# divideon/xvc

Hardware: AMD Instinct MI355X
Metric: hot-path frame passes/s (TZ + sub-pel ME, MC, transform + RDOQ + dequant + inverse, deblock, pad, PSNR parts), bit-exact vs the reference's classes (higher is better)
Workload: dtype u16; 1 GPU; 1920x1080 yuv420p 30fps synthetic, QP 32, internal bitdepth 10, 16x16 CUs, TZ range 96, RDOQ (RdoQuant::QuantRdo + CoeffSignHideRdo, picture-initial CABAC contexts); cus_per_picture=8160, parallelism=3 independent picture chains in flight

## Files before the change

### include/xvcgpu.h

```cpp
#ifndef XVCGPU_H_
#define XVCGPU_H_

#include "xvcgpu_types.h"

#ifdef __cplusplus
extern "C" {
#endif

typedef enum xvcgpu_status {
  XVCGPU_OK = 0,
  XVCGPU_INVALID_ARGUMENT = 10,
  XVCGPU_NO_DEVICE = 20,
  XVCGPU_OUT_OF_MEMORY = 30,
  XVCGPU_DEVICE_ERROR = 40,
  XVCGPU_UNSUPPORTED = 50
} xvcgpu_status;

typedef struct xvcgpu_ctx xvcgpu_ctx;
typedef struct xvcgpu_picture xvcgpu_picture;

xvcgpu_status xvcgpu_create(int device, xvcgpu_ctx **out);
void xvcgpu_destroy(xvcgpu_ctx *ctx);
const char *xvcgpu_last_error(const xvcgpu_ctx *ctx);
const char *xvcgpu_version(void);
// ... 146 lines not shown
                                  const xvcgpu_mc_lic_block *d_blocks, int n);

xvcgpu_status xvcgpu_inter_pred_batch(xvcgpu_ctx *ctx, const xvcgpu_picture *const *refs,
                                      int n_refs, const xvcgpu_picture *rec,
                                      xvcgpu_picture *pred,
                                      const xvcgpu_inter_block *d_blocks, int n);

xvcgpu_status xvcgpu_inter_pred_batch_to(xvcgpu_ctx *ctx, const xvcgpu_picture *const *refs,
                                         int n_refs, const xvcgpu_picture *rec,
                                         xvcgpu_picture *scratch,
                                         const xvcgpu_inter_block *d_blocks,
                                         const xvcgpu_block_pos *d_dst, int n);

xvcgpu_status xvcgpu_copy_blocks(xvcgpu_ctx *ctx, const xvcgpu_picture *src,
                                 xvcgpu_picture *dst, const xvcgpu_copy_block *d_blocks,
                                 int n);

xvcgpu_status xvcgpu_inv_transform_cu_order(xvcgpu_ctx *ctx, xvcgpu_picture *rec,
                                            const xvcgpu_tx_block *d_blocks, int n_cus,
                                            const int16_t *d_levels,
                                            const uint32_t *d_level_offsets,
                                            const int32_t *d_nnz);

xvcgpu_status xvcgpu_mc_affine_batch(xvcgpu_ctx *ctx, const xvcgpu_picture *ref,
                                     xvcgpu_picture *pred,
                                     const xvcgpu_mc_affine_block *d_blocks, int n);

xvcgpu_status xvcgpu_mc_bipred_batch(xvcgpu_ctx *ctx, const xvcgpu_picture *ref0,
                                     const xvcgpu_picture *ref1,
                                     xvcgpu_picture *pred,
                                     const xvcgpu_mc_bi_block *d_blocks, int n);

xvcgpu_status xvcgpu_bipred_search(xvcgpu_ctx *ctx, const xvcgpu_picture *orig,
                                   const xvcgpu_picture *ref_other,
                                   const xvcgpu_picture *ref_search,
                                   const xvcgpu_bi_block *d_jobs, int n,
                                   xvcgpu_me_result *d_results,
                                   int max_block_size);
xvcgpu_status xvcgpu_bipred_search_lic(xvcgpu_ctx *ctx, const xvcgpu_picture *orig,
                                       const xvcgpu_picture *ref_other,
                                       const xvcgpu_picture *ref_search,
                                       const xvcgpu_picture *rec,
                                       const xvcgpu_bi_block *d_jobs,
                                       const xvcgpu_mc_lic_block *d_neighbours, int n,
                                       xvcgpu_me_result *d_results, int max_block_size);

// ... 54 lines not shown
                                          xvcgpu_cu_info *d_cus);
xvcgpu_status xvcgpu_fwd_from_me_classify_prove(
    xvcgpu_ctx *ctx, const xvcgpu_picture *orig, const xvcgpu_picture *ref, xvcgpu_picture *pred,
    const xvcgpu_me_block *d_blocks, const xvcgpu_me_result *d_results, int n, int qp_y, int qp_c,
    int ref_poc, int16_t *d_coeffs, const uint32_t *d_coeff_offsets, size_t n_coeffs,
    int16_t *d_levels, int32_t *d_nnz, xvcgpu_cu_info *d_cus,
    const xvcgpu_rdoq_contexts *d_contexts, const xvcgpu_rdoq_params *d_params);
xvcgpu_status xvcgpu_quant_rdo_classified_batch(xvcgpu_ctx *ctx, int bitdepth,
                                                const xvcgpu_tx_block *d_blocks, int n,
                                                const int16_t *d_coeffs,
                                                const uint32_t *d_offsets, size_t n_coeffs,
                                                int16_t *d_levels, int32_t *d_nnz,
                                                const xvcgpu_rdoq_contexts *d_contexts,
                                                const xvcgpu_rdoq_params *d_params,
                                                xvcgpu_cu_info *d_cus);

xvcgpu_status xvcgpu_quant_rdo_reserve(xvcgpu_ctx *ctx, int n, size_t n_coeffs);

#define XVCGPU_PROVE_ZERO_AUTO_BLOCKS 65536
#define XVCGPU_PROVE_ZERO_AUTO_QP 30
xvcgpu_status xvcgpu_quant_rdo_set_prove_zero(xvcgpu_ctx *ctx, int mode);

xvcgpu_status xvcgpu_quant_rdo_class_counts(xvcgpu_ctx *ctx, int32_t out[3]);
xvcgpu_status xvcgpu_quant_rdo_set_four_lane_only(xvcgpu_ctx *ctx, int on);

xvcgpu_status xvcgpu_recon_from_me(xvcgpu_ctx *ctx, const xvcgpu_picture *orig,
                                   const xvcgpu_picture *ref, xvcgpu_picture *rec,
                                   const xvcgpu_me_block *d_blocks,
                                   const xvcgpu_me_result *d_results, int n,
                                   int qp_y, int qp_c, int intra_pic, int ref_poc,
                                   int32_t *d_nnz, xvcgpu_cu_info *d_cus);

xvcgpu_status xvcgpu_fwd_from_me(xvcgpu_ctx *ctx, const xvcgpu_picture *orig,
                                 const xvcgpu_picture *ref, xvcgpu_picture *pred,
                                 const xvcgpu_me_block *d_blocks,
                                 const xvcgpu_me_result *d_results, int n, int16_t *d_coeffs,
                                 const uint32_t *d_coeff_offsets);
xvcgpu_status xvcgpu_recon_from_me_rdoq(xvcgpu_ctx *ctx, const xvcgpu_picture *orig,
                                        const xvcgpu_picture *ref, xvcgpu_picture *rec,
                                        const xvcgpu_me_block *d_blocks,
                                        const xvcgpu_me_result *d_results, int n,
                                        int qp_y, int qp_c, int tx_flags, int ref_poc,
                                        int32_t *d_nnz, xvcgpu_cu_info *d_cus,
                                        const xvcgpu_rdoq_contexts *d_contexts,
                                        const xvcgpu_rdoq_params *d_params);

// ... 202 lines not shown
```

### xvc_amd/api.py

```python
import ctypes as C
import os

import numpy as np

HERE = os.path.dirname(os.path.abspath(__file__))
LIB_PATH = os.environ.get("XVCGPU_LIB") or os.path.join(HERE, "libxvcgpu.so")

BORDER_LUMA = 128
BORDER_CHROMA = 64
ME_FULLPEL = 1
ME_SUBPEL = 2
ME_LIC_JOBS = 4
ME_HINT_SQ16 = 8
ME_ONLY_SQ16 = 16

METRIC_SSD, METRIC_SATD, METRIC_SATD_ACONLY, METRIC_SAD, METRIC_SAD_FAST, \
    METRIC_SAD_ACONLY, METRIC_SAD_ACONLY_FAST, METRIC_STRUCTURAL_SSD = range(8)
TX_DEFAULT, TX_DCT2, TX_DCT5, TX_DCT8, TX_DST1, TX_DST7 = range(6)

CU_DTYPE = np.dtype([("x", "<u2"), ("y", "<u2"), ("w", "u1"), ("h", "u1"),
                     ("intra", "u1"), ("cbf_luma", "u1"), ("qp_y", "i1"),
                     ("qp_c", "i1"), ("ref_idx0", "i1"), ("reserved", "i1"),
                     ("ref_poc", "<i4", (2,)), ("mv", "<i4", (2, 4, 2))])
ME_DTYPE = np.dtype([("x", "<i2"), ("y", "<i2"), ("w", "u1"), ("h", "u1"),
# ... 129 lines not shown
    "xvcgpu_picture_download", "xvcgpu_picture_upload_padded",
    "xvcgpu_picture_download_padded", "xvcgpu_picture_plane",
    "xvcgpu_picture_copy", "xvcgpu_pad_border", "xvcgpu_metric_batch", "xvcgpu_mc_metric_batch",
    "xvcgpu_me_search", "xvcgpu_me_search_sized", "xvcgpu_mc_batch", "xvcgpu_mc_from_me",
    "xvcgpu_mc_bipred_batch", "xvcgpu_bipred_search", "xvcgpu_mc_affine_batch", "xvcgpu_mc_lic_batch",
    "xvcgpu_affine_me_batch",
    "xvcgpu_me_search_refs",
    "xvcgpu_bipred_search_refs",
    "xvcgpu_mc_metric_batch_refs",
    "xvcgpu_affine_me_batch_refs",
    "xvcgpu_cu_info_from_me", "xvcgpu_recon_from_me", "xvcgpu_residual_batch",
    "xvcgpu_fwd_transform_batch", "xvcgpu_inv_transform_batch",
    "xvcgpu_deblock", "xvcgpu_deblock_rows", "xvcgpu_deblock_pad_ssd", "xvcgpu_picture_ssd", "xvcgpu_picture_ssd_rows",
    "xvcgpu_picture_import", "xvcgpu_picture_export", "xvcgpu_picture_crc",
    "xvcgpu_variance_map", "xvcgpu_histogram_distance",
    "xvcgpu_intra_pred_batch", "xvcgpu_intra_satd_batch", "xvcgpu_intra_recon_batch",
    "xvcgpu_intra_select_modes", "xvcgpu_frame_pass", "xvcgpu_frame_pass_multi", "xvcgpu_copy_segments",
    "xvcgpu_get_transform_matrix", "xvcgpu_inter_pred_batch", "xvcgpu_deblock_tree",
    "xvcgpu_residual_rdoq_batch", "xvcgpu_quant_rdo_batch", "xvcgpu_recon_from_me_rdoq",
    "xvcgpu_quant_rdo_reserve", "xvcgpu_quant_rdo_class_counts", "xvcgpu_quant_rdo_set_prove_zero",
    "xvcgpu_tx_eval_batch", "xvcgpu_root_cbf_batch", "xvcgpu_bipred_search_lic",
    "xvcgpu_inter_pred_batch_to", "xvcgpu_copy_blocks", "xvcgpu_intra_recon_waves",
    "xvcgpu_host_alloc", "xvcgpu_host_free", "xvcgpu_memcpy_h2d_async",
    "xvcgpu_inv_transform_cu_order",
    "xvcgpu_fwd_from_me_classify", "xvcgpu_fwd_from_me_classify_prove", "xvcgpu_quant_rdo_classified_batch",
    "xvcgpu_event_create", "xvcgpu_event_destroy", "xvcgpu_event_record", "xvcgpu_event_wait",
    "xvcgpu_event_synchronize", "xvcgpu_comm_unique_id", "xvcgpu_comm_create",
    "xvcgpu_comm_destroy", "xvcgpu_comm_world", "xvcgpu_comm_rank", "xvcgpu_comm_wait_event",
    "xvcgpu_comm_record_event", "xvcgpu_comm_sync", "xvcgpu_comm_group_begin",
    "xvcgpu_comm_group_end", "xvcgpu_comm_send_picture", "xvcgpu_comm_recv_picture",
    "xvcgpu_comm_send_rows", "xvcgpu_comm_recv_rows", "xvcgpu_comm_all_reduce_sum_u64",
    "xvcgpu_comm_send_bytes", "xvcgpu_comm_recv_bytes", "xvcgpu_inv_transform_dist_batch",
    "xvcgpu_fwd_from_me", "xvcgpu_output_bytes", "xvcgpu_picture_convert_to",
    "xvcgpu_me_plan_create", "xvcgpu_me_plan_counts", "xvcgpu_me_plan_destroy",
    "xvcgpu_me_search_planned", "xvcgpu_frame_pass_planned",
]

_vp = C.c_void_p
_pd = C.c_ssize_t
_lib = None


class XvcGpuError(RuntimeError):
    pass


class MePlan:
# ... 105 lines not shown
        "xvcgpu_intra_pred_batch": [_vp, _vp, _vp, _vp, C.c_int],
        "xvcgpu_intra_satd_batch": [_vp, _vp, _vp, _vp, C.c_int, _vp, C.c_int],
        "xvcgpu_intra_recon_batch": [_vp, _vp, _vp, _vp, _vp, C.c_int, _vp, _vp, _vp],
        "xvcgpu_intra_select_modes": [_vp, _vp, _vp, C.c_int, _vp, _vp, _vp, C.c_int],
        "xvcgpu_frame_pass": [_vp, C.POINTER(FramePassArgs), C.c_int],
        "xvcgpu_frame_pass_multi": [C.POINTER(_vp), C.POINTER(C.POINTER(FramePassArgs)), C.c_int,
                                    C.c_int],
        "xvcgpu_copy_segments": [_vp, _vp, C.c_int],
        "xvcgpu_get_transform_matrix": [C.c_int, C.c_int, _vp],
        "xvcgpu_inter_pred_batch": [_vp, C.POINTER(_vp), C.c_int, _vp, _vp, _vp, C.c_int],
        "xvcgpu_residual_rdoq_batch": [_vp, _vp, _vp, _vp, _vp, C.c_int, _vp, _vp, _vp, _vp, _vp],
        "xvcgpu_recon_from_me_rdoq": [_vp, _vp, _vp, _vp, _vp, _vp, C.c_int, C.c_int, C.c_int,
                                      C.c_int, C.c_int, _vp, _vp, _vp, _vp],
        "xvcgpu_quant_rdo_reserve": [_vp, C.c_int, C.c_size_t],
        "xvcgpu_quant_rdo_class_counts": [_vp, _vp],
        "xvcgpu_quant_rdo_set_prove_zero": [_vp, C.c_int],
        "xvcgpu_quant_rdo_set_four_lane_only": [_vp, C.c_int],
        "xvcgpu_tx_eval_batch": [_vp, _vp, C.c_int, _vp, _vp],
        "xvcgpu_inter_pred_batch_to": [_vp, _vp, C.c_int, _vp, _vp, _vp, _vp, C.c_int],
        "xvcgpu_copy_blocks": [_vp, _vp, _vp, _vp, C.c_int],
        "xvcgpu_host_alloc": [_vp, C.c_size_t, C.POINTER(_vp)],
        "xvcgpu_host_free": [_vp, _vp],
        "xvcgpu_inv_transform_cu_order": [_vp, _vp, _vp, C.c_int, _vp, _vp, _vp],
        "xvcgpu_memcpy_h2d_async": [_vp, _vp, _vp, C.c_size_t],
        "xvcgpu_memcpy_d2h_async": [_vp, _vp, _vp, C.c_size_t],
        "xvcgpu_upload_ahead": [_vp, _vp, _vp, C.c_size_t, _vp, _vp],
        "xvcgpu_eval_dist_batch": [_vp, _vp, _vp, _vp, C.c_int, _vp, C.c_int, _vp],
        "xvcgpu_cs_start_fold": [_vp, _vp, C.c_int, C.c_int, _vp, _vp, _vp, _vp, _vp, C.c_int, C.c_int],
        "xvcgpu_cs_uni_fold": [_vp, _vp, C.c_int, C.c_int, _vp, _vp, _vp, _vp, _vp],
        "xvcgpu_cs_bi_fold": [_vp, _vp, C.c_int, C.c_int, _vp, _vp, _vp, _vp],
        "xvcgpu_cs_merge_fold": [_vp, _vp, C.c_int, C.c_int, _vp, _vp, _vp, _vp],
        "xvcgpu_residual_rdoq_batch_at": [_vp, _vp, _vp, _vp, _vp, C.c_int, _vp, _vp, _vp, _vp, _vp, _vp,
                                          C.c_int, _vp, C.c_int, _vp],
        "xvcgpu_intra_recon_waves": [_vp, _vp, _vp, _vp, _vp, _vp, C.c_int, _vp, _vp, _vp],
        "xvcgpu_bipred_search_lic": [_vp, _vp, _vp, _vp, _vp, _vp, _vp, C.c_int, _vp, C.c_int],
        "xvcgpu_root_cbf_batch": [_vp, _vp, C.c_int, _vp],
        "xvcgpu_quant_rdo_batch": [_vp, C.c_int, _vp, C.c_int, _vp, _vp, C.c_size_t, _vp, _vp,
                                   _vp, _vp],
        "xvcgpu_deblock_pad_ssd": [_vp, _vp, _vp, _vp, _vp, C.c_int, _vp, C.c_int, C.c_int,
                                   C.c_int, C.c_int, C.c_int, _vp],
        "xvcgpu_deblock_tree": [_vp, _vp, _vp, C.c_int, _vp, C.c_int, C.c_int, C.c_int,
                                C.c_int, C.c_int, C.c_int],
        "xvcgpu_event_create": [_vp, C.POINTER(_vp)],
        "xvcgpu_event_record": [_vp, _vp],
        "xvcgpu_event_wait": [_vp, _vp],
        "xvcgpu_event_synchronize": [_vp],
# ... 882 lines not shown
```

### xvc_amd/csrc/k_multi.h

```cpp
#ifndef XVCGPU_K_MULTI_H_
#define XVCGPU_K_MULTI_H_

#include "k_me2.h"
#include "k_misc.h"
#include "k_rdoq.h"
#include "k_recon.h"
#include "k_tail.h"
#include "k_tx.h"
#include "k_tx2.h"

struct ReconMultiArgs {
  PicView orig, ref, rec;
  const xvcgpu_me_block *blocks;
  const xvcgpu_me_result *results;
  int n_cus, qp_y, qp_c, ref_poc;
  int32_t *nnz_out;
  xvcgpu_cu_info *cus;
  int16_t *coeffs;
  const uint32_t *coeff_off;
};
template <bool FWD>
__global__ void __launch_bounds__(256)
recon_from_me_multi_kernel(MultiArgs<ReconMultiArgs> m, const int16_t *tx_tables,
                           const int16_t *tx_tables_t, TxTableLayout lay) {
// ... 4 lines not shown
                                        FwdClassify());
}

struct RdoqMultiArgs {
  const xvcgpu_tx_block *blocks;
  int n;
  const int16_t *coeffs;
  const uint32_t *d_off;
  int16_t *levels;
  int32_t *nnz_out;
  RdoqLists l;
  const xvcgpu_rdoq_contexts *rq_ctx;
  const xvcgpu_rdoq_params *rq_prm;
};
__global__ void __launch_bounds__(256)
rdoq_classify_multi_kernel(MultiArgs<RdoqMultiArgs> m, int bd) {
  const RdoqMultiArgs &a = m.a[blockIdx.y];
  rdoq_classify_kernel_body(bd, a.blocks, a.n, a.coeffs, a.d_off, a.levels, a.nnz_out, a.l);
}
__global__ void __launch_bounds__(1024)
rdoq_compact_multi_kernel(MultiArgs<RdoqMultiArgs> m) {
  const RdoqMultiArgs &a = m.a[blockIdx.y];
  rdoq_compact_kernel_body(a.n, a.l);
}
__global__ void __launch_bounds__(64, RDOQ4_MIN_WAVES)
quant_rdo_packed4_multi_kernel(MultiArgs<RdoqMultiArgs> m, int bd, int g16) {
  const RdoqMultiArgs &a = m.a[blockIdx.y];
  quant_rdo_packed4_kernel_body(bd, a.blocks, a.l, g16, a.coeffs, a.d_off, a.levels, a.nnz_out,
                                a.rq_ctx, a.rq_prm, nullptr);
}
__global__ void __launch_bounds__(64, RDOQ_MIN_WAVES)
quant_rdo_packed_multi_kernel(MultiArgs<RdoqMultiArgs> m, int bd) {
  const RdoqMultiArgs &a = m.a[blockIdx.y];
  quant_rdo_packed_kernel_body(bd, a.blocks, a.l, a.coeffs, a.d_off, a.levels, a.nnz_out,
                               a.rq_ctx, a.rq_prm, nullptr);
}

struct InvMultiArgs {
  PicView pred, rec;
  const xvcgpu_tx_block *blocks;
  int n;
  int16_t *levels;
  const uint32_t *level_off;
  int32_t *nnz;
};
__global__ void __launch_bounds__(64 * TX2_WAVES)
// ... 49 lines not shown
```

### xvc_amd/csrc/k_rdoq.h

```cpp
#ifndef XVCGPU_K_RDOQ_H_
#define XVCGPU_K_RDOQ_H_

#include "dev_common.h"
#include "dev_tables.h"
#include "k_me.h"
#include "k_me2.h"
#include "xvcgpu_internal.h"

__constant__ uint32_t kEntropyBits[128] = {
#include "entropy_bits.inc"
};

#define RQ_BYPASS 32768u
__device__ uint32_t gEntropyBits[128];

#ifdef XVCGPU_TRACE
__device__ unsigned long long g_rq_trace[4096][16];
#define RQ_TRACE(k)                                                          \
  do {                                                                       \
    if (threadIdx.x == 0 && blockIdx.x < 4096)                               \
      g_rq_trace[blockIdx.x][k] = __builtin_amdgcn_s_memtime();              \
  } while (0)
#define RQ_TRACE_RT(k)                                                       \
  do {                                                                       \
// ... 1362 lines not shown
    }
  }
}

__global__ void __launch_bounds__(1024)
rdoq_count_kernel(int n, RdoqLists l) {
  __shared__ int wsum[3][16];
  int cnt[3];
  rdoq_chunk_counts(n, l, cnt);
  const int t = threadIdx.x;
#pragma unroll
  for (int k = 0; k < 3; k++) {
    const int v = wave_reduce_add_i32(cnt[k]);
    if ((t & 63) == 0) wsum[k][t >> 6] = v;
  }
  __syncthreads();
  if (t < 3) {
    int v = 0;
    for (int w = 0; w < 16; w++) v += wsum[t][w];
    l.part[4 * blockIdx.x + t] = v;
  }
}

__global__ void __launch_bounds__(1024)
rdoq_scatter_kernel(int n, RdoqLists l) {
  __shared__ int part[3][1024];
  __shared__ int base[3];
  const int t = threadIdx.x, b = blockIdx.x;
  {
    int v[3] = {0, 0, 0};
    for (int j = t; j < b; j += 1024) {
      v[0] += l.part[4 * j];
      v[1] += l.part[4 * j + 1];
      v[2] += l.part[4 * j + 2];
    }
#pragma unroll
    for (int k = 0; k < 3; k++) {
      const int w = wave_reduce_add_i32(v[k]);
      if ((t & 63) == 0) part[k][t >> 6] = w;
    }
    __syncthreads();
    if (t < 3) {
      int sum = 0;
      for (int w = 0; w < 16; w++) sum += part[t][w];
      base[t] = sum;
    }
    __syncthreads();
  }
  int cnt[3];
  rdoq_chunk_counts(n, l, cnt);
  int inc[3];
#pragma unroll
  for (int k = 0; k < 3; k++) {
    int v = cnt[k];
#pragma unroll
    for (int d = 1; d < 64; d <<= 1) {
      const int o = __shfl_up(v, d, 64);
// ... 15 lines not shown
#pragma unroll
      for (int d = 1; d < 16; d <<= 1) {
        const int o = __shfl_up(v, d, 64);
        if (t >= d) v += o;
      }
      if (t < 16) part[k][16 + t] = v;
    }
  }
  __syncthreads();
  const int bs[3] = {b0, b1, b2};
  int pos[3];
#pragma unroll
  for (int k = 0; k < 3; k++)
    pos[k] = bs[k] + inc[k] - cnt[k] + ((t >> 6) ? part[k][16 + (t >> 6) - 1] : 0);
  const int i = b * RDOQ_CHUNK + 4 * t;
  if (i < n) {
    const uint32_t v = reinterpret_cast<const uint32_t *>(l.cls)[i >> 2];
#pragma unroll
    for (int k = 0; k < 4; k++) {
      const int c = (int)(signed char)(v >> (8 * k));
      if (i + k < n && c >= 0) l.list[c][pos[c]++] = i + k;
    }
  }
  if (b == (int)gridDim.x - 1 && t == 1023)
    for (int k = 0; k < 3; k++) l.count[k] = bs[k] + part[k][16 + 15];
}

template <int G, int NSB>
struct RdoqPackedLds {
  static constexpr int GROUPS = 64 / G;
  static constexpr int MAXC = 16 * NSB;
  static constexpr int MAXSB = NSB;
  static constexpr int MAXR = RQ_PADDED(MAXC);
  static constexpr int MAXT = RQ_CF_PADDED(MAXC);
  alignas(8) long long sb_code_cost[GROUPS][MAXSB];
  alignas(8) int16_t cf[GROUPS][MAXT], lv[GROUPS][MAXT];
  alignas(8) int16_t wl[GROUPS][RQ_WL(MAXC)];
  long long fcs[NSB == 64 ? 256 : 1];
  unsigned short rate_up[GROUPS][MAXR];
  alignas(8) unsigned ctx_bits[2 * sizeof(xvcgpu_rdoq_contexts)];
  unsigned csbf_bits[GROUPS][MAXSB];
  unsigned char csbf[GROUPS][MAXSB], sb_live[GROUPS][MAXSB], sb_dcz[GROUPS][MAXSB];
  unsigned char sb_of_scan[GROUPS][NSB == 4 ? MAXSB : MAXSB * 4];
  unsigned lp_bits[32];
};

struct RqTileCf {
  const int16_t *p;
// ... 273 lines not shown
```

### xvc_amd/csrc/k_tx2.h

```cpp
#ifndef XVCGPU_K_TX2_H_
#define XVCGPU_K_TX2_H_

#include "dev_common.h"
#include "dev_tables.h"
#include "k_me.h"
#include "k_me2.h"
#include "k_tx.h"
#include "xvcgpu_internal.h"

#define TX2_WAVES 4

typedef short tx2_v2s __attribute__((ext_vector_type(2)));

struct __attribute__((aligned(16))) Tx2Shared {
  int16_t r[256];
  int16_t t[256];
  int16_t c[256];
};

__device__ __forceinline__ int tx2_dot2(uint32_t a, uint32_t b, int acc) {
  return __builtin_amdgcn_sdot2(__builtin_bit_cast(tx2_v2s, a),
                                __builtin_bit_cast(tx2_v2s, b), acc, false);
}

// ... 395 lines not shown
  if (job >= n) return;
  const int ci = job >> 1;
  if (!(job & 1)) {
    const int bi = 3 * ci;
    if (nnz_out[bi] == 0) return;
    const xvcgpu_tx_block b = blocks[bi];
    if (!tx_small_job(b)) return;
    const PlaneView pc = rec.c[0];
    tx2_job<TX_MODE_INV, 64, false>(s, b, bi, rec.bd, pc, pc.p + (ptrdiff_t)b.y * pc.stride + b.x,
                                    pc.stride, pc, levels, level_off, nnz_out, tx_tables,
                                    tx_tables_t, lay);
    return;
  }
  if (nnz_out[3 * ci + 1] == 0 && nnz_out[3 * ci + 2] == 0) return;
  const int g = ME2_LANE >> 5, bi = 3 * ci + 1 + g;
  const xvcgpu_tx_block b = blocks[bi];
  if (!tx_small_job(b) || b.w * b.h > 64) return;
  const PlaneView pc = g ? rec.c[2] : rec.c[1];
  tx2_job<TX_MODE_INV, 32, false>(s, b, bi, rec.bd, pc, pc.p + (ptrdiff_t)b.y * pc.stride + b.x,
                                  pc.stride, pc, levels, level_off, nnz_out, tx_tables,
                                  tx_tables_t, lay, nullptr, g * 128);
}

template <int MODE, bool RDOQ = false>
__global__ void __launch_bounds__(64 * TX2_WAVES)
residual_wave_kernel(PicView orig, PicView pred, PicView rec, const xvcgpu_tx_block *blocks, int n, int16_t *levels, const uint32_t *level_off, int32_t *nnz_out, const int16_t *tx_tables, const int16_t *tx_tables_t, TxTableLayout lay, const xvcgpu_rdoq_contexts *rq_ctx = nullptr, const xvcgpu_rdoq_params *rq_prm = nullptr, unsigned long long *dist_out = nullptr) {
  residual_wave_kernel_body<MODE, RDOQ>(orig, pred, rec, blocks, n, levels, level_off, nnz_out, tx_tables, tx_tables_t, lay, rq_ctx, rq_prm, dist_out);
}

template <int MODE, bool RDOQ>
__device__ __forceinline__ void
residual_cu_body(const PicView &orig, const PicView &pred, const PicView &rec, const xvcgpu_tx_block *blocks, int n,
                   int16_t *levels, const uint32_t *level_off, int32_t *nnz_out,
                   const int16_t *tx_tables, const int16_t *tx_tables_t, TxTableLayout lay,
                   const xvcgpu_rdoq_contexts *rq_ctx, const xvcgpu_rdoq_params *rq_prm,
                   const xvcgpu_block_pos *src_pos, const xvcgpu_eval_cand *ecands, int n_head,
                   uint64_t *eout, int strength) {
  struct Big {
    TxShared s;
    RdoqShared<RDOQ ? 1024 : 4> rq;
  };
  struct Small {
    Tx2Shared s;
    RdoqShared<256> rq;
  };
  constexpr size_t kBytes = sizeof(Big) > sizeof(Small) ? sizeof(Big) : sizeof(Small);
// ... 65 lines not shown
```

### xvc_amd/csrc/xvcgpu.hip

```cpp
#include <hip/hip_runtime.h>
#include <stdlib.h>
#include <stdio.h>
#include <string.h>

#include <algorithm>
#include <new>
#include <vector>

#include "k_deblock.h"
#include "k_tail.h"
#include "k_me.h"
#include "k_me2.h"
#include "k_me_plan.h"
#include "k_metric.h"
#include "k_misc.h"
#include "k_pad.h"
#include "k_tx.h"
#include "k_tx2.h"
#include "k_recon.h"
#include "k_bipred.h"
#include "k_stats.h"
#include "k_output.h"
#include "k_intra.h"
#include "k_affine_me.h"
// ... 1349 lines not shown
}

xvcgpu_status xvcgpu_quant_rdo_set_four_lane_only(xvcgpu_ctx *ctx, int on) {
  if (!ctx) return XVCGPU_INVALID_ARGUMENT;
  ctx->rdoq_four_lane_only = on ? 1 : 0;
  return XVCGPU_OK;
}

xvcgpu_status xvcgpu_quant_rdo_reserve(xvcgpu_ctx *ctx, int n, size_t n_coeffs) {
  if (!ctx || n < 0) return XVCGPU_INVALID_ARGUMENT;
  return ensure_rdoq_scratch(ctx, n, n_coeffs);
}

static RdoqLists rdoq_lists_of(xvcgpu_ctx *ctx) {
  const int cap = ctx->rdoq_lists_cap;
  RdoqLists l;
  l.count = ctx->d_rdoq_lists;
  for (int c = 0; c < 3; c++) l.list[c] = ctx->d_rdoq_lists + 4 + (size_t)c * cap;
  l.cls = reinterpret_cast<signed char *>(ctx->d_rdoq_lists + 4 + 3 * (size_t)cap);
  l.part = ctx->d_rdoq_lists + 4 + 4 * (size_t)cap;
  return l;
}

static xvcgpu_status quant_rdo_launch(xvcgpu_ctx *ctx, int bitdepth,
                                      const xvcgpu_tx_block *d_blocks, int n,
                                      const int16_t *d_coeffs, const uint32_t *d_offsets,
                                      size_t n_coeffs, int16_t *d_levels, int32_t *d_nnz,
                                      const xvcgpu_rdoq_contexts *d_contexts,
                                      const xvcgpu_rdoq_params *d_params, bool classified,
                                      xvcgpu_cu_info *d_cu_patch = nullptr) {
  if (!ctx || n < 0 || bitdepth < 8 || bitdepth > 12 ||
      (n && (!d_blocks || !d_coeffs || !d_offsets || !d_levels || !d_contexts || !d_params ||
             !n_coeffs)))
    return XVCGPU_INVALID_ARGUMENT;
  if (n == 0) return XVCGPU_OK;
  {
    const xvcgpu_status st_ = ensure_rdoq_scratch(ctx, n, n_coeffs);
    if (st_ != XVCGPU_OK) return st_;
  }
  const RdoqLists l = rdoq_lists_of(ctx);
  if (!classified)
    hipLaunchKernelGGL(rdoq_classify_kernel, dim3((n + 3) / 4), dim3(256), 0, ctx->stream,
                       bitdepth, d_blocks, n, d_coeffs, d_offsets, d_levels, d_nnz, l);
  const int qp_hint = classified ? ctx->rdoq_qp_hint : -1;
  const bool proved_already = classified && ctx->rdoq_classified_proved;
  if (!proved_already &&
      (ctx->rdoq_prove_zero > 0 ||
       (ctx->rdoq_prove_zero < 0 && n >= XVCGPU_PROVE_ZERO_AUTO_BLOCKS &&
        (qp_hint < 0 || qp_hint >= XVCGPU_PROVE_ZERO_AUTO_QP))))
    hipLaunchKernelGGL(rdoq_prove_zero_kernel, dim3((n + RQ_PROVE_BLOCKS - 1) / RQ_PROVE_BLOCKS),
                       dim3(256), 0, ctx->stream,
                       bitdepth, d_blocks, n, d_coeffs, d_offsets, d_levels, d_nnz, d_contexts,
                       d_params, l);
  {
    const int chunks = (n + RDOQ_CHUNK - 1) / RDOQ_CHUNK;
    hipLaunchKernelGGL(rdoq_count_kernel, dim3(chunks), dim3(1024), 0, ctx->stream, n, l);
    hipLaunchKernelGGL(rdoq_scatter_kernel, dim3(chunks), dim3(1024), 0, ctx->stream, n, l);
  }
  static const int grid16 = [] {
    const char *e = getenv("XVCGPU_RDOQ_GRID16");
    const int v = e ? atoi(e) : 0;
    return v > 0 ? v : RDOQ_GRID16;
  }();
  const int g16 = std::min(n, grid16), g4 = std::min((n + 3) / 4, RDOQ_GRID4),
            g64 = std::min(n, RDOQ_GRID64);
  const bool four_only = ctx->rdoq_four_lane_only != 0;
  hipLaunchKernelGGL(quant_rdo_packed4_kernel, dim3(g16 + g4), dim3(64), 0, ctx->stream,
                     bitdepth, d_blocks, l, g16, d_coeffs, d_offsets, d_levels, d_nnz,
                     d_contexts, d_params, d_cu_patch, four_only ? ctx->h_rdoq_misuse : nullptr);
  if (!four_only)
    hipLaunchKernelGGL(quant_rdo_packed_kernel, dim3(g64), dim3(64), 0, ctx->stream,
                       bitdepth, d_blocks, l, d_coeffs, d_offsets, d_levels, d_nnz,
                       d_contexts, d_params, d_cu_patch);
  CHECK_LAUNCH(ctx, "quant_rdo_batch");
  return XVCGPU_OK;
}

xvcgpu_status xvcgpu_quant_rdo_batch(xvcgpu_ctx *ctx, int bitdepth,
                                     const xvcgpu_tx_block *d_blocks, int n,
                                     const int16_t *d_coeffs, const uint32_t *d_offsets,
                                     size_t n_coeffs, int16_t *d_levels, int32_t *d_nnz,
// ... 93 lines not shown
  if (n == 0) return XVCGPU_OK;
  launch_residual<TX_MODE_INV>(ctx, pred->v, pred->v, rec->v, d_blocks, n,
                               const_cast<int16_t *>(d_levels), d_level_offsets,
                               const_cast<int32_t *>(d_nnz));
  CHECK_LAUNCH(ctx, "inv_transform_batch");
  return XVCGPU_OK;
}

xvcgpu_status xvcgpu_inv_transform_cu_order(xvcgpu_ctx *ctx, xvcgpu_picture *rec,
                                            const xvcgpu_tx_block *d_blocks, int n_cus,
                                            const int16_t *d_levels,
                                            const uint32_t *d_level_offsets,
                                            const int32_t *d_nnz) {
  if (!ctx || !rec || n_cus < 0 ||
      (n_cus && (!d_blocks || !d_levels || !d_level_offsets || !d_nnz)))
    return XVCGPU_INVALID_ARGUMENT;
  if (n_cus == 0) return XVCGPU_OK;
  const int n_wg = (2 * n_cus + TX2_WAVES - 1) / TX2_WAVES;
  hipLaunchKernelGGL(inv_cu_pairs_kernel, dim3((n_wg + 7) / 8 * 8), dim3(64 * TX2_WAVES), 0,
                     ctx->stream, rec->v, d_blocks, n_cus, const_cast<int16_t *>(d_levels),
                     d_level_offsets, const_cast<int32_t *>(d_nnz), ctx->d_tx_tables,
                     ctx->d_tx_tables_t, xvcgpu_tx_layout());
  CHECK_LAUNCH(ctx, "inv_transform_cu_order");
  return XVCGPU_OK;
}

xvcgpu_status xvcgpu_inv_transform_dist_batch(xvcgpu_ctx *ctx, const xvcgpu_picture *orig,
                                              const xvcgpu_picture *pred, xvcgpu_picture *rec,
                                              const xvcgpu_tx_block *d_blocks, int n,
                                              const int16_t *d_levels,
                                              const uint32_t *d_level_offsets,
                                              const int32_t *d_nnz, uint64_t *d_dist) {
  if (!ctx || !orig || !pred || !rec || n < 0 ||
      (n && (!d_blocks || !d_levels || !d_level_offsets || !d_nnz || !d_dist)))
    return XVCGPU_INVALID_ARGUMENT;
  if (orig->w != pred->w || orig->h != pred->h || orig->bd != pred->bd)
    return fail(ctx, XVCGPU_INVALID_ARGUMENT, "picture mismatch");
  if (n == 0) return XVCGPU_OK;
  launch_residual<TX_MODE_INV>(ctx, orig->v, pred->v, rec->v, d_blocks, n,
                               const_cast<int16_t *>(d_levels), d_level_offsets,
                               const_cast<int32_t *>(d_nnz),
                               reinterpret_cast<unsigned long long *>(d_dist));
  CHECK_LAUNCH(ctx, "inv_transform_dist_batch");
  return XVCGPU_OK;
}

// ... 777 lines not shown
        st = xvcgpu_quant_rdo_set_four_lane_only(ctx, 1);
      if (st == XVCGPU_OK)
        st = classified
                 ? xvcgpu_quant_rdo_classified_batch(ctx, a->rec->bd, a->d_tx, a->n_tx,
                                                     a->d_coeffs, a->d_level_off, a->n_coeffs,
                                                     a->d_levels, a->d_nnz, a->d_rdoq_contexts,
                                                     a->d_rdoq_params, a->d_cus_own)
                 : xvcgpu_quant_rdo_batch(ctx, a->rec->bd, a->d_tx, a->n_tx, a->d_coeffs,
                                          a->d_level_off, a->n_coeffs, a->d_levels, a->d_nnz,
                                          a->d_rdoq_contexts, a->d_rdoq_params);
      ctx->rdoq_four_lane_only = four_before;
      if (st == XVCGPU_OK) {
        if (!a->d_tx || !a->d_levels || !a->d_level_off || !a->d_nnz) {
          st = XVCGPU_INVALID_ARGUMENT;
        } else if (a->n_tx > 0) {
          const PicView &pv = in_place ? rec->v : a->pred->v;
          if (ctx->hi_stream && fused_tail && in_place) {
            HIP_TRY(ctx, hipEventRecord(ctx->ev_hi_in, ctx->stream));
            HIP_TRY(ctx, hipStreamWaitEvent(ctx->hi_stream, ctx->ev_hi_in, 0));
            main_stream = ctx->stream;
            ctx->stream = ctx->hi_stream;
          }
          if (in_place) {
            st = xvcgpu_inv_transform_cu_order(ctx, rec, a->d_tx, a->n_cus, a->d_levels,
                                               a->d_level_off, a->d_nnz);
          } else {
            launch_residual<TX_MODE_INV>(ctx, pv, pv, rec->v, a->d_tx, a->n_tx, a->d_levels,
                                         a->d_level_off, a->d_nnz, nullptr, false);
          }
          CHECK_LAUNCH(ctx, "inv_transform_batch");
        }
      }
      if (st == XVCGPU_OK && !(classified && a->d_cus_own))
        st = xvcgpu_cu_info_from_me(ctx, a->d_me, a->d_results, a->d_nnz, a->d_luma_tx_index,
                                    a->n_cus, a->qp_y, a->qp_c, a->ref_poc, a->d_cus_own);
    } else if (a->d_rdoq_params)
      st = xvcgpu_recon_from_me_rdoq(ctx, a->orig, a->ref, rec, a->d_me, a->d_results,
                                     a->n_cus, a->qp_y, a->qp_c, 0, a->ref_poc, a->d_nnz,
                                     a->d_cus_own, a->d_rdoq_contexts, a->d_rdoq_params);
    else
      st = xvcgpu_recon_from_me(ctx, a->orig, a->ref, rec, a->d_me, a->d_results, a->n_cus,
                                a->qp_y, a->qp_c, 0, a->ref_poc, a->d_nnz, a->d_cus_own);
    if (st != XVCGPU_OK) return st;
  }
  if (fused_tail)
    return xvcgpu_deblock_pad_ssd(ctx, a->scratch_rec, a->rec, a->orig, a->d_cus, a->n_cus_total,
                                  a->d_cu_map, a->map_stride, 0, 0, 0, a->shift_bitdepth,
                                  a->d_ssd);
// ... 145 lines not shown
    MultiArgs<RdoqMultiArgs> q;
    for (int i = 0; i < n; i++) {
      const xvcgpu_frame_pass_args *a = args[i];
      xvcgpu_ctx *c = ctxs[i];
      const xvcgpu_status st = ensure_rdoq_scratch(c, a->n_tx, a->n_coeffs);
      if (st != XVCGPU_OK) return st;
      const int cap = c->rdoq_lists_cap;
      RdoqMultiArgs &k = q.a[i];
      k.blocks = a->d_tx;
      k.n = a->n_tx;
      k.coeffs = a->d_coeffs;
      k.d_off = a->d_level_off;
      k.levels = a->d_levels;
      k.nnz_out = a->d_nnz;
      k.l.count = c->d_rdoq_lists;
      for (int cl = 0; cl < 3; cl++) k.l.list[cl] = c->d_rdoq_lists + 4 + (size_t)cl * cap;
      k.l.cls = reinterpret_cast<signed char *>(c->d_rdoq_lists + 4 + 3 * (size_t)cap);
      k.rq_ctx = a->d_rdoq_contexts;
      k.rq_prm = a->d_rdoq_params;
    }
    const int bd = args[0]->rec->bd;
    hipLaunchKernelGGL(rdoq_classify_multi_kernel, dim3((max_tx + 3) / 4, n), dim3(256), 0,
                       ctx->stream, q, bd);
    hipLaunchKernelGGL(rdoq_compact_multi_kernel, dim3(1, n), dim3(1024), 0, ctx->stream, q);
    const int g16 = std::min(max_tx, RDOQ_GRID16),
              g4 = std::min((max_tx + 3) / 4, RDOQ_GRID4), g64 = std::min(max_tx, RDOQ_GRID64);
    hipLaunchKernelGGL(quant_rdo_packed4_multi_kernel, dim3(g16 + g4, n), dim3(64), 0,
                       ctx->stream, q, bd, g16);
    hipLaunchKernelGGL(quant_rdo_packed_multi_kernel, dim3(g64, n), dim3(64), 0,
                       ctx->stream, q, bd);
    MultiArgs<InvMultiArgs> v;
    for (int i = 0; i < n; i++) {
      const xvcgpu_frame_pass_args *a = args[i];
      InvMultiArgs &k = v.a[i];
      k.pred = a->scratch_rec->v;
      k.rec = a->scratch_rec->v;
      k.blocks = a->d_tx;
      k.n = a->n_tx;
      k.levels = a->d_levels;
      k.level_off = a->d_level_off;
      k.nnz = a->d_nnz;
    }
    const int n_wg = (max_tx + TX2_WAVES - 1) / TX2_WAVES;
    hipLaunchKernelGGL(inv_wave_multi_kernel, dim3((n_wg + 7) / 8 * 8, n), dim3(64 * TX2_WAVES), 0,
                       ctx->stream, v, ctx->d_tx_tables, ctx->d_tx_tables_t, lay);
    hipLaunchKernelGGL(inv_general_multi_kernel, dim3((max_tx + TX_THREADS - 1) / TX_THREADS, n),
                       dim3(TX_THREADS), 0, ctx->stream, v, ctx->d_tx_tables, lay);
// ... 486 lines not shown
```

Measured before the change: 8616 frame passes/s.

## Build RDOQ class lists in one launch and run inverse transform from lists

Result: no change. 8577 frame passes/s (-0.4%).

```diff
diff --git a/include/xvcgpu.h b/include/xvcgpu.h
--- a/include/xvcgpu.h
+++ b/include/xvcgpu.h
@@ -192,6 +192,12 @@
                                             const uint32_t *d_level_offsets,
                                             const int32_t *d_nnz);
 
+xvcgpu_status xvcgpu_inv_transform_listed(xvcgpu_ctx *ctx, xvcgpu_picture *rec,
+                                          const xvcgpu_tx_block *d_blocks, int n_cus,
+                                          const int16_t *d_levels,
+                                          const uint32_t *d_level_offsets,
+                                          const int32_t *d_nnz);
+
 xvcgpu_status xvcgpu_mc_affine_batch(xvcgpu_ctx *ctx, const xvcgpu_picture *ref,
                                      xvcgpu_picture *pred,
                                      const xvcgpu_mc_affine_block *d_blocks, int n);
@@ -292,6 +298,9 @@
 xvcgpu_status xvcgpu_quant_rdo_set_prove_zero(xvcgpu_ctx *ctx, int mode);
 
 xvcgpu_status xvcgpu_quant_rdo_class_counts(xvcgpu_ctx *ctx, int32_t out[3]);
+xvcgpu_status xvcgpu_quant_rdo_lists_from_classes(xvcgpu_ctx *ctx, const int8_t *d_cls, int n,
+                                                  int form, int32_t *d_lists,
+                                                  int32_t *d_counts);
 xvcgpu_status xvcgpu_quant_rdo_set_four_lane_only(xvcgpu_ctx *ctx, int on);
 
 xvcgpu_status xvcgpu_recon_from_me(xvcgpu_ctx *ctx, const xvcgpu_picture *orig,
diff --git a/xvc_amd/api.py b/xvc_amd/api.py
--- a/xvc_amd/api.py
+++ b/xvc_amd/api.py
@@ -175,7 +175,8 @@
     "xvcgpu_tx_eval_batch", "xvcgpu_root_cbf_batch", "xvcgpu_bipred_search_lic",
     "xvcgpu_inter_pred_batch_to", "xvcgpu_copy_blocks", "xvcgpu_intra_recon_waves",
     "xvcgpu_host_alloc", "xvcgpu_host_free", "xvcgpu_memcpy_h2d_async",
-    "xvcgpu_inv_transform_cu_order",
+    "xvcgpu_inv_transform_cu_order", "xvcgpu_inv_transform_listed",
+    "xvcgpu_quant_rdo_lists_from_classes",
     "xvcgpu_fwd_from_me_classify", "xvcgpu_fwd_from_me_classify_prove", "xvcgpu_quant_rdo_classified_batch",
     "xvcgpu_event_create", "xvcgpu_event_destroy", "xvcgpu_event_record", "xvcgpu_event_wait",
     "xvcgpu_event_synchronize", "xvcgpu_comm_unique_id", "xvcgpu_comm_create",
@@ -327,6 +328,8 @@
         "xvcgpu_host_alloc": [_vp, C.c_size_t, C.POINTER(_vp)],
         "xvcgpu_host_free": [_vp, _vp],
         "xvcgpu_inv_transform_cu_order": [_vp, _vp, _vp, C.c_int, _vp, _vp, _vp],
+        "xvcgpu_inv_transform_listed": [_vp, _vp, _vp, C.c_int, _vp, _vp, _vp],
+        "xvcgpu_quant_rdo_lists_from_classes": [_vp, _vp, C.c_int, C.c_int, _vp, _vp],
         "xvcgpu_memcpy_h2d_async": [_vp, _vp, _vp, C.c_size_t],
         "xvcgpu_memcpy_d2h_async": [_vp, _vp, _vp, C.c_size_t],
         "xvcgpu_upload_ahead": [_vp, _vp, _vp, C.c_size_t, _vp, _vp],
diff --git a/xvc_amd/csrc/k_multi.h b/xvc_amd/csrc/k_multi.h
--- a/xvc_amd/csrc/k_multi.h
+++ b/xvc_amd/csrc/k_multi.h
@@ -50,6 +50,11 @@
 rdoq_compact_multi_kernel(MultiArgs<RdoqMultiArgs> m) {
   const RdoqMultiArgs &a = m.a[blockIdx.y];
   rdoq_compact_kernel_body(a.n, a.l);
+}
+__global__ void __launch_bounds__(1024)
+rdoq_lists_multi_kernel(MultiArgs<RdoqMultiArgs> m) {
+  const RdoqMultiArgs &a = m.a[blockIdx.y];
+  rdoq_scatter_kernel_body<true>(a.n, a.l);
 }
 __global__ void __launch_bounds__(64, RDOQ4_MIN_WAVES)
 quant_rdo_packed4_multi_kernel(MultiArgs<RdoqMultiArgs> m, int bd, int g16) {
diff --git a/xvc_amd/csrc/k_rdoq.h b/xvc_amd/csrc/k_rdoq.h
--- a/xvc_amd/csrc/k_rdoq.h
+++ b/xvc_amd/csrc/k_rdoq.h
@@ -1408,17 +1408,39 @@
   }
 }
 
-__global__ void __launch_bounds__(1024)
-rdoq_scatter_kernel(int n, RdoqLists l) {
+#ifndef RDOQ_ONE_LAUNCH_CHUNKS
+#define RDOQ_ONE_LAUNCH_CHUNKS 32
+#endif
+template <bool ONE>
+__device__ __forceinline__ void rdoq_scatter_kernel_body(int n, RdoqLists l) {
   __shared__ int part[3][1024];
   __shared__ int base[3];
   const int t = threadIdx.x, b = blockIdx.x;
+  const int chunks = (n + RDOQ_CHUNK - 1) / RDOQ_CHUNK;
+  if (b >= chunks) {
+    if (n == 0 && b == 0 && t < 3) l.count[t] = 0;
+    return;
+  }
   {
     int v[3] = {0, 0, 0};
-    for (int j = t; j < b; j += 1024) {
-      v[0] += l.part[4 * j];
-      v[1] += l.part[4 * j + 1];
-      v[2] += l.part[4 * j + 2];
+    if (ONE) {
+      const uint32_t *cw = reinterpret_cast<const uint32_t *>(l.cls) + t;
+      for (int j = 0; j < b; j++) {
+        const uint32_t w = cw[j * (RDOQ_CHUNK / 4)];
+#pragma unroll
+        for (int k = 0; k < 4; k++) {
+          const int c = (int)(signed char)(w >> (8 * k));
+          v[0] += c == 0;
+          v[1] += c == 1;
+          v[2] += c == 2;
+        }
+      }
+    } else {
+      for (int j = t; j < b; j += 1024) {
+        v[0] += l.part[4 * j];
+        v[1] += l.part[4 * j + 1];
+        v[2] += l.part[4 * j + 2];
+      }
     }
 #pragma unroll
     for (int k = 0; k < 3; k++) {
@@ -1480,8 +1502,18 @@
       if (i + k < n && c >= 0) l.list[c][pos[c]++] = i + k;
     }
   }
-  if (b == (int)gridDim.x - 1 && t == 1023)
+  if (b == chunks - 1 && t == 1023)
     for (int k = 0; k < 3; k++) l.count[k] = bs[k] + part[k][16 + 15];
+}
+
+__global__ void __launch_bounds__(1024)
+rdoq_scatter_kernel(int n, RdoqLists l) {
+  rdoq_scatter_kernel_body<false>(n, l);
+}
+
+__global__ void __launch_bounds__(1024)
+rdoq_lists_kernel(int n, RdoqLists l) {
+  rdoq_scatter_kernel_body<true>(n, l);
 }
 
 template <int G, int NSB>
diff --git a/xvc_amd/csrc/k_tx2.h b/xvc_amd/csrc/k_tx2.h
--- a/xvc_amd/csrc/k_tx2.h
+++ b/xvc_amd/csrc/k_tx2.h
@@ -441,6 +441,66 @@
                                   tx_tables_t, lay, nullptr, g * 128);
 }
 
+__device__ __forceinline__ void inv_listed_kernel_body(
+    const PicView &rec, const xvcgpu_tx_block *blocks, const RdoqLists &l, int g_full,
+    int16_t *levels, const uint32_t *level_off, int32_t *nnz_out, const int16_t *tx_tables,
+    const int16_t *tx_tables_t, const TxTableLayout &lay) {
+  __shared__ Tx2Shared s_all[TX2_WAVES];
+  const int wave = (int)(threadIdx.x >> 6);
+  Tx2Shared &s = s_all[wave];
+  if ((int)blockIdx.x < g_full) {
+    const int n1 = l.count[1], n = n1 + l.count[2];
+    for (int j = (int)blockIdx.x * TX2_WAVES + wave; j < n; j += g_full * TX2_WAVES) {
+      const int bi =
+          __builtin_amdgcn_readfirstlane(j < n1 ? l.list[1][j] : l.list[2][j - n1]);
+      if (nnz_out[bi] == 0) continue;
+      const xvcgpu_tx_block b = blocks[bi];
+      if (!tx_small_job(b)) continue;
+      const PlaneView pc = b.comp == 0 ? rec.c[0] : (b.comp == 1 ? rec.c[1] : rec.c[2]);
+      const uint16_t *at = pc.p + (ptrdiff_t)b.y * pc.stride + b.x;
+      if (b.w == 16 && b.h == 16)
+        tx2_job<TX_MODE_INV, 64, false, 16, 16>(s, b, bi, rec.bd, pc, at, pc.stride, pc, levels,
+                                                level_off, nnz_out, tx_tables, tx_tables_t, lay);
+      else
+        tx2_job<TX_MODE_INV, 64, false>(s, b, bi, rec.bd, pc, at, pc.stride, pc, levels,
+                                        level_off, nnz_out, tx_tables, tx_tables_t, lay);
+      wave_sync();
+    }
+    return;
+  }
+  const int g_half = (int)gridDim.x - g_full, n0 = l.count[0];
+  const int g = ME2_LANE >> 5;
+  for (int j = ((int)blockIdx.x - g_full) * TX2_WAVES + wave; 2 * j < n0;
+       j += g_half * TX2_WAVES) {
+    const int e = 2 * j + g;
+    const int bi = e < n0 ? l.list[0][e] : -1;
+    if (bi >= 0 && nnz_out[bi] != 0) {
+      const xvcgpu_tx_block b = blocks[bi];
+      if (tx_small_job(b) && b.w * b.h <= 64) {
+        const PlaneView pc = b.comp == 0 ? rec.c[0] : (b.comp == 1 ? rec.c[1] : rec.c[2]);
+        const uint16_t *at = pc.p + (ptrdiff_t)b.y * pc.stride + b.x;
+        if (b.w == 8 && b.h == 8)
+          tx2_job<TX_MODE_INV, 32, false, 8, 8>(s, b, bi, rec.bd, pc, at, pc.stride, pc, levels,
+                                                level_off, nnz_out, tx_tables, tx_tables_t, lay,
+                                                nullptr, g * 128);
+        else
+          tx2_job<TX_MODE_INV, 32, false>(s, b, bi, rec.bd, pc, at, pc.stride, pc, levels,
+                                          level_off, nnz_out, tx_tables, tx_tables_t, lay,
+                                          nullptr, g * 128);
+      }
+    }
+    wave_sync();
+  }
+}
+
+__global__ void __launch_bounds__(64 * TX2_WAVES)
+inv_listed_kernel(PicView rec, const xvcgpu_tx_block *blocks, RdoqLists l, int g_full,
+                  int16_t *levels, const uint32_t *level_off, int32_t *nnz_out,
+                  const int16_t *tx_tables, const int16_t *tx_tables_t, TxTableLayout lay) {
+  inv_listed_kernel_body(rec, blocks, l, g_full, levels, level_off, nnz_out, tx_tables,
+                         tx_tables_t, lay);
+}
+
 template <int MODE, bool RDOQ = false>
 __global__ void __launch_bounds__(64 * TX2_WAVES)
 residual_wave_kernel(PicView orig, PicView pred, PicView rec, const xvcgpu_tx_block *blocks, int n, int16_t *levels, const uint32_t *level_off, int32_t *nnz_out, const int16_t *tx_tables, const int16_t *tx_tables_t, TxTableLayout lay, const xvcgpu_rdoq_contexts *rq_ctx = nullptr, const xvcgpu_rdoq_params *rq_prm = nullptr, unsigned long long *dist_out = nullptr) {
diff --git a/xvc_amd/csrc/xvcgpu.hip b/xvc_amd/csrc/xvcgpu.hip
--- a/xvc_amd/csrc/xvcgpu.hip
+++ b/xvc_amd/csrc/xvcgpu.hip
@@ -1395,6 +1395,24 @@
   return l;
 }
 
+static int rdoq_one_launch_chunks() {
+  static const int v = [] {
+    const char *e = getenv("XVCGPU_RDOQ_ONE_LAUNCH_CHUNKS");
+    return e ? atoi(e) : RDOQ_ONE_LAUNCH_CHUNKS;
+  }();
+  return v;
+}
+
+static void launch_rdoq_lists(xvcgpu_ctx *ctx, int n, const RdoqLists &l, int form) {
+  const int chunks = std::max(1, (n + RDOQ_CHUNK - 1) / RDOQ_CHUNK);
+  if (form == 1 || (form == 0 && chunks <= rdoq_one_launch_chunks())) {
+    hipLaunchKernelGGL(rdoq_lists_kernel, dim3(chunks), dim3(1024), 0, ctx->stream, n, l);
+    return;
+  }
+  hipLaunchKernelGGL(rdoq_count_kernel, dim3(chunks), dim3(1024), 0, ctx->stream, n, l);
+  hipLaunchKernelGGL(rdoq_scatter_kernel, dim3(chunks), dim3(1024), 0, ctx->stream, n, l);
+}
+
 static xvcgpu_status quant_rdo_launch(xvcgpu_ctx *ctx, int bitdepth,
                                       const xvcgpu_tx_block *d_blocks, int n,
                                       const int16_t *d_coeffs, const uint32_t *d_offsets,
@@ -1425,11 +1443,7 @@
                        dim3(256), 0, ctx->stream,
                        bitdepth, d_blocks, n, d_coeffs, d_offsets, d_levels, d_nnz, d_contexts,
                        d_params, l);
-  {
-    const int chunks = (n + RDOQ_CHUNK - 1) / RDOQ_CHUNK;
-    hipLaunchKernelGGL(rdoq_count_kernel, dim3(chunks), dim3(1024), 0, ctx->stream, n, l);
-    hipLaunchKernelGGL(rdoq_scatter_kernel, dim3(chunks), dim3(1024), 0, ctx->stream, n, l);
-  }
+  launch_rdoq_lists(ctx, n, l, 0);
   static const int grid16 = [] {
     const char *e = getenv("XVCGPU_RDOQ_GRID16");
     const int v = e ? atoi(e) : 0;
@@ -1569,6 +1583,59 @@
                      d_level_offsets, const_cast<int32_t *>(d_nnz), ctx->d_tx_tables,
                      ctx->d_tx_tables_t, xvcgpu_tx_layout());
   CHECK_LAUNCH(ctx, "inv_transform_cu_order");
+  return XVCGPU_OK;
+}
+
+#ifndef INV_LISTED_GRID_FULL
+#define INV_LISTED_GRID_FULL 2048
+#endif
+#ifndef INV_LISTED_GRID_HALF
+#define INV_LISTED_GRID_HALF 512
+#endif
+
+xvcgpu_status xvcgpu_inv_transform_listed(xvcgpu_ctx *ctx, xvcgpu_picture *rec,
+                                          const xvcgpu_tx_block *d_blocks, int n_cus,
+                                          const int16_t *d_levels,
+                                          const uint32_t *d_level_offsets,
+                                          const int32_t *d_nnz) {
+  if (!ctx || !rec || n_cus < 0 ||
+      (n_cus && (!d_blocks || !d_levels || !d_level_offsets || !d_nnz)))
+    return XVCGPU_INVALID_ARGUMENT;
+  if (n_cus == 0) return XVCGPU_OK;
+  if (!ctx->d_rdoq_lists || (long long)ctx->rdoq_lists_cap < 3ll * n_cus)
+    return fail(ctx, XVCGPU_INVALID_ARGUMENT,
+                "inv_transform_listed: no class lists of a quantiser batch of 3 * n_cus blocks");
+  const int n = 3 * n_cus;
+  const int g_full = std::min((n + TX2_WAVES - 1) / TX2_WAVES, INV_LISTED_GRID_FULL);
+  const int g_half = std::min((n + 2 * TX2_WAVES - 1) / (2 * TX2_WAVES), INV_LISTED_GRID_HALF);
+  hipLaunchKernelGGL(inv_listed_kernel, dim3(g_full + g_half), dim3(64 * TX2_WAVES), 0,
+                     ctx->stream, rec->v, d_blocks, rdoq_lists_of(ctx), g_full,
+                     const_cast<int16_t *>(d_levels), d_level_offsets,
+                     const_cast<int32_t *>(d_nnz), ctx->d_tx_tables, ctx->d_tx_tables_t,
+                     xvcgpu_tx_layout());
+  CHECK_LAUNCH(ctx, "inv_transform_listed");
+  return XVCGPU_OK;
+}
+
+xvcgpu_status xvcgpu_quant_rdo_lists_from_classes(xvcgpu_ctx *ctx, const int8_t *d_cls, int n,
+                                                  int form, int32_t *d_lists,
+                                                  int32_t *d_counts) {
+  if (!ctx || n < 0 || form < 0 || form > 2 || !d_counts || (n && (!d_cls || !d_lists)))
+    return XVCGPU_INVALID_ARGUMENT;
+  {
+    const xvcgpu_status st = ensure_rdoq_scratch(ctx, std::max(n, 1), 0);
+    if (st != XVCGPU_OK) return st;
+  }
+  const RdoqLists l = rdoq_lists_of(ctx);
+  if (n)
+    HIP_TRY(ctx, hipMemcpyAsync(l.cls, d_cls, (size_t)n, hipMemcpyDeviceToDevice, ctx->stream));
+  launch_rdoq_lists(ctx, n, l, form);
+  CHECK_LAUNCH(ctx, "quant_rdo_lists_from_classes");
+  for (int c = 0; c < 3 && n; c++)
+    HIP_TRY(ctx, hipMemcpyAsync(d_lists + (size_t)c * n, l.list[c], sizeof(int32_t) * (size_t)n,
+                                hipMemcpyDeviceToDevice, ctx->stream));
+  HIP_TRY(ctx, hipMemcpyAsync(d_counts, l.count, 3 * sizeof(int32_t), hipMemcpyDeviceToDevice,
+                              ctx->stream));
   return XVCGPU_OK;
 }
 
@@ -2392,8 +2459,8 @@
             ctx->stream = ctx->hi_stream;
           }
           if (in_place) {
-            st = xvcgpu_inv_transform_cu_order(ctx, rec, a->d_tx, a->n_cus, a->d_levels,
-                                               a->d_level_off, a->d_nnz);
+            st = xvcgpu_inv_transform_listed(ctx, rec, a->d_tx, a->n_cus, a->d_levels,
+                                             a->d_level_off, a->d_nnz);
           } else {
             launch_residual<TX_MODE_INV>(ctx, pv, pv, rec->v, a->d_tx, a->n_tx, a->d_levels,
                                          a->d_level_off, a->d_nnz, nullptr, false);
@@ -2585,7 +2652,14 @@
     const int bd = args[0]->rec->bd;
     hipLaunchKernelGGL(rdoq_classify_multi_kernel, dim3((max_tx + 3) / 4, n), dim3(256), 0,
                        ctx->stream, q, bd);
-    hipLaunchKernelGGL(rdoq_compact_multi_kernel, dim3(1, n), dim3(1024), 0, ctx->stream, q);
+    {
+      const int chunks = (max_tx + RDOQ_CHUNK - 1) / RDOQ_CHUNK;
+      if (chunks <= rdoq_one_launch_chunks())
+        hipLaunchKernelGGL(rdoq_lists_multi_kernel, dim3(std::max(1, chunks), n), dim3(1024), 0,
+                           ctx->stream, q);
+      else
+        hipLaunchKernelGGL(rdoq_compact_multi_kernel, dim3(1, n), dim3(1024), 0, ctx->stream, q);
+    }
     const int g16 = std::min(max_tx, RDOQ_GRID16),
               g4 = std::min((max_tx + 3) / 4, RDOQ_GRID4), g64 = std::min(max_tx, RDOQ_GRID64);
     hipLaunchKernelGGL(quant_rdo_packed4_multi_kernel, dim3(g16 + g4, n), dim3(64), 0,
```
